# tencent-ailab/V-Express

Hardware: AMD Instinct MI355X
Metric: decoded frames/sec at 512x512, 25 DDIM steps (higher is better)
Workload: dtype bf16; 1 GPU; 512x512, 16 frames (1 window(s) of 16, overlap 4), 25 DDIM steps, CFG 3.5, random-init UNet3D + ReferenceNet banks + sd-vae-ft-mse decode; frames=16, windows=1, parallelism=window x CFG-half units over 1 GPU(s)

## Files before the change

v-express_amd/csrc/vx_attn.hip:

```cpp
#include "vx_common.h"
#include <stdio.h>
#include "../../include/vexpress_hip.h"

#include <stdlib.h>

#include <type_traits>

namespace {

struct AttnParams {
  const bf16_t* q; int ldq;
  const bf16_t* k; int ldk;
  const bf16_t* vt; int vt_pitch;
  bf16_t* out; int ldo;
  int batch, heads, n_q, n_kv, d, q_per_kv;
  float c;
  const float* kmax;
};

__device__ __forceinline__ int k_lds_off(int slab, int key, int grp) {
  return slab * 4096 + key * 64 + ((grp ^ ((0 - (key >> 2)) & 3)) << 4);
}
__device__ __forceinline__ int v_lds_off(int row, int chunk) { return row * 128 + ((chunk ^ ((row >> 1) & 7)) << 4); }

// ... 697 lines not shown
  };
  if (wide && (p.heads % 8) == 0 && KK * (p.f <= 16 ? 1 : 2) <= 6) {
    dim3 grid((unsigned)((waves + 7) / 8));
    name(p.f <= 16 ? 0 : 1, p.f <= 16 ? 1 : 2, 8);
    if (p.f <= 16) hipLaunchKernelGGL((temporal_attn_kernel<KK, DT, 1, 8>), grid, dim3(512), 0, stream, p);
    else hipLaunchKernelGGL((temporal_attn_kernel<KK, DT, 2, 8>), grid, dim3(512), 0, stream, p);
    return vx_check_launch("vx_temporal_attention");
  }
  dim3 grid((unsigned)((waves + 3) / 4));
  name(p.f <= 16 ? 2 : 3, p.f <= 16 ? 1 : 2, 4);
  if (p.f <= 16) hipLaunchKernelGGL((temporal_attn_kernel<KK, DT, 1, 4>), grid, dim3(256), 0, stream, p);
  else hipLaunchKernelGGL((temporal_attn_kernel<KK, DT, 2, 4>), grid, dim3(256), 0, stream, p);
  return vx_check_launch("vx_temporal_attention");
}

constexpr int SKV_MAX = 16;

__global__ __launch_bounds__(256) void small_kv_attn_kernel(const bf16_t* __restrict__ q, int ldq,
                                                            const bf16_t* __restrict__ kv, int ldkv, int v_off,
                                                            bf16_t* __restrict__ out, int ldo, int n_q, int n_kv,
                                                            int heads, int d, float c) {
  extern __shared__ __attribute__((aligned(16))) char smem[];
  bf16_t* kvs = reinterpret_cast<bf16_t*>(smem);
  const int C = heads * d;
  const int b = blockIdx.y;
  const int tid = threadIdx.x;
  const int cch = C >> 3;
  for (int idx = tid; idx < n_kv * 2 * cch; idx += 256) {
    int j = idx / (2 * cch), rem = idx % (2 * cch);
    int which = rem / cch, ch = (rem % cch) * 8;
    const bf16_t* src = kv + ((size_t)b * n_kv + j) * ldkv + (which ? v_off : 0) + ch;
    *reinterpret_cast<uint4*>(kvs + ((size_t)(j * 2 + which)) * C + ch) = *reinterpret_cast<const uint4*>(src);
  }
  __syncthreads();
  const long item = (long)blockIdx.x * 256 + tid;
  if (item >= (long)n_q * heads) return;
  const int h = (int)(item % heads);
  const int tok = (int)(item / heads);
  const bf16_t* qp = q + ((size_t)b * n_q + tok) * ldq + h * d;
  float sc[SKV_MAX];
#pragma unroll
  for (int j = 0; j < SKV_MAX; ++j) sc[j] = 0.f;
  for (int ch = 0; ch < d; ch += 8) {
    float qv[8];
    unpack_bf16x8(*reinterpret_cast<const uint4*>(qp + ch), qv);
#pragma unroll
    for (int j = 0; j < SKV_MAX; ++j) {
      if (j < n_kv) {
        float kvv[8];
        unpack_bf16x8(*reinterpret_cast<const uint4*>(kvs + (size_t)(j * 2) * C + h * d + ch), kvv);
#pragma unroll
        for (int e = 0; e < 8; ++e) sc[j] = fmaf(qv[e], kvv[e], sc[j]);
      }
    }
  }
  float mx = -INFINITY;
#pragma unroll
  for (int j = 0; j < SKV_MAX; ++j)
    if (j < n_kv) mx = fmaxf(mx, sc[j]);
  float den = 0.f;
#pragma unroll
  for (int j = 0; j < SKV_MAX; ++j) {
    float pv = (j < n_kv) ? __builtin_amdgcn_exp2f((sc[j] - mx) * c) : 0.f;
    sc[j] = pv;
    den += pv;
  }
  const float inv = 1.0f / den;
  bf16_t* op = out + ((size_t)b * n_q + tok) * ldo + h * d;
  for (int ch = 0; ch < d; ch += 8) {
    float acc[8] = {0.f, 0.f, 0.f, 0.f, 0.f, 0.f, 0.f, 0.f};
#pragma unroll
    for (int j = 0; j < SKV_MAX; ++j) {
      if (j < n_kv) {
        float vv[8];
        unpack_bf16x8(*reinterpret_cast<const uint4*>(kvs + (size_t)(j * 2 + 1) * C + h * d + ch), vv);
#pragma unroll
        for (int e = 0; e < 8; ++e) acc[e] = fmaf(sc[j], vv[e], acc[e]);
      }
    }
#pragma unroll
    for (int e = 0; e < 8; ++e) acc[e] *= inv;
    *reinterpret_cast<uint4*>(op + ch) = pack_bf16x8(acc);
  }
}

__global__ __launch_bounds__(256) void key_norm_max_kernel(const bf16_t* __restrict__ k, int ldk, int heads, int n_kv,
                                                           int d, float* __restrict__ out) {
  __shared__ float red[256];
  const int bh = blockIdx.x, b = bh / heads, h = bh - b * heads;
  const bf16_t* base = k + (size_t)b * n_kv * ldk + h * d;
  const int chunks = d >> 3;
  float best = 0.f;
  for (int key = threadIdx.x; key < n_kv; key += 256) {
    const bf16_t* row = base + (size_t)key * ldk;
    float ss = 0.f;
    for (int c = 0; c < chunks; ++c) {
      float f[8];
      unpack_bf16x8(*reinterpret_cast<const uint4*>(row + 8 * c), f);
#pragma unroll
      for (int e = 0; e < 8; ++e) ss = fmaf(f[e], f[e], ss);
    }
    best = fmaxf(best, ss);
  }
  red[threadIdx.x] = best;
  __syncthreads();
  for (int s = 128; s > 0; s >>= 1) {
    if ((int)threadIdx.x < s) red[threadIdx.x] = fmaxf(red[threadIdx.x], red[threadIdx.x + s]);
    __syncthreads();
  }
  if (threadIdx.x == 0) out[bh] = sqrtf(red[0]);
}

constexpr int KNM8_KEYS = 256;
__global__ __launch_bounds__(256) void key_norm_max8_kernel(const bf16_t* __restrict__ k, int ldk, int n_kv, int d,
                                                            float* __restrict__ out) {
  __shared__ float red[4][8];
  const int b = blockIdx.y, key0 = blockIdx.x * KNM8_KEYS;
  const int lane = threadIdx.x & 63, wave = threadIdx.x >> 6, h = lane & 7;
  const bf16_t* base = k + (size_t)b * n_kv * ldk + h * d;
  const int chunks = d >> 3;
  float best = 0.f;
  for (int kk = wave * 8 + (lane >> 3); kk < KNM8_KEYS; kk += 32) {
    const int key = min(key0 + kk, n_kv - 1);
    const bf16_t* row = base + (size_t)key * ldk;
    float ss = 0.f;
    for (int c = 0; c < chunks; ++c) {
      float f[8];
      unpack_bf16x8(*reinterpret_cast<const uint4*>(row + 8 * c), f);
#pragma unroll
      for (int e = 0; e < 8; ++e) ss = fmaf(f[e], f[e], ss);
    }
    best = fmaxf(best, ss);
  }
  best = fmaxf(best, __shfl_xor(best, 8, 64));
  best = fmaxf(best, __shfl_xor(best, 16, 64));
  best = fmaxf(best, __shfl_xor(best, 32, 64));
  if (lane < 8) red[wave][lane] = best;
  __syncthreads();
  if (threadIdx.x < 8) {
    const float m = fmaxf(fmaxf(red[0][threadIdx.x], red[1][threadIdx.x]), fmaxf(red[2][threadIdx.x], red[3][threadIdx.x]));
    atomicMax(reinterpret_cast<unsigned int*>(out) + b * 8 + threadIdx.x, __float_as_uint(sqrtf(m)));
  }
}

int attention_impl(const void* q, int ldq, const void* k, int ldk, const void* vt, int vt_pitch, void* out, int ldo,
                   int batch, int heads, int n_q, int n_kv, int head_dim, int q_per_kv, float scale,
                   const float* key_norm_max, hipStream_t stream);

}

int vx_attn3_variant();
int vx_attn3_launch(const void* q, int ldq, const void* k, int ldk, const void* vt, int vt_pitch, void* out, int ldo,
                    int batch, int heads, int n_q, int n_kv, int q_per_kv, float c, const float* kmax,
                    hipStream_t stream);

extern "C" int vx_key_norm_max(const void* k, int ldk, int kv_batches, int heads, int n_kv, int head_dim, float* out,
                               void* stream) {
  VX_REQUIRE(k && out, "vx_key_norm_max: null pointer");
  VX_REQUIRE(kv_batches > 0 && heads > 0 && n_kv > 0 && head_dim > 0 && (head_dim % 8) == 0 && (ldk % 8) == 0,
             "vx_key_norm_max: bad sizes (head_dim=%d ldk=%d)", head_dim, ldk);
  static int v8 = -1;
  if (v8 < 0) {
    const char* e = getenv("VX_KNM8");
    v8 = !(e && atoi(e) == 0);
  }
  if (v8 && heads == 8 && n_kv >= 2 * KNM8_KEYS && kv_batches <= 65535) {
    if (hipMemsetAsync(out, 0, (size_t)kv_batches * heads * sizeof(float), (hipStream_t)stream) != hipSuccess) {
      vx_set_error("vx_key_norm_max: hipMemsetAsync failed");
      return VX_ERR_HIP;
    }
    hipLaunchKernelGGL(key_norm_max8_kernel, dim3((n_kv + KNM8_KEYS - 1) / KNM8_KEYS, kv_batches), dim3(256), 0,
                       (hipStream_t)stream, (const bf16_t*)k, ldk, n_kv, head_dim, out);
    return vx_check_launch("vx_key_norm_max");
  }
  hipLaunchKernelGGL(key_norm_max_kernel, dim3(kv_batches * heads), dim3(256), 0, (hipStream_t)stream,
                     (const bf16_t*)k, ldk, heads, n_kv, head_dim, out);
  return vx_check_launch("vx_key_norm_max");
}

extern "C" int vx_attention(const void* q, int ldq, const void* k, int ldk, const void* vt, int vt_pitch, void* out,
                            int ldo, int batch, int heads, int n_q, int n_kv, int head_dim, int q_per_kv,
                            float scale, void* stream) {
  return attention_impl(q, ldq, k, ldk, vt, vt_pitch, out, ldo, batch, heads, n_q, n_kv, head_dim, q_per_kv, scale,
                        nullptr, (hipStream_t)stream);
}

extern "C" int vx_attention_bounded(const void* q, int ldq, const void* k, int ldk, const void* vt, int vt_pitch,
                                    void* out, int ldo, int batch, int heads, int n_q, int n_kv, int head_dim,
                                    int q_per_kv, float scale, const float* key_norm_max, void* stream) {
  VX_REQUIRE(key_norm_max != nullptr, "vx_attention_bounded: null key_norm_max");
  return attention_impl(q, ldq, k, ldk, vt, vt_pitch, out, ldo, batch, heads, n_q, n_kv, head_dim, q_per_kv, scale,
                        key_norm_max, (hipStream_t)stream);
}

namespace {
int attention_impl(const void* q, int ldq, const void* k, int ldk, const void* vt, int vt_pitch, void* out, int ldo,
                   int batch, int heads, int n_q, int n_kv, int head_dim, int q_per_kv, float scale,
                   const float* key_norm_max, hipStream_t stream) {
  VX_REQUIRE(q && k && vt && out, "vx_attention: null pointer");
  VX_REQUIRE(batch > 0 && heads > 0 && n_q > 0 && n_kv > 0 && q_per_kv > 0 && (batch % q_per_kv) == 0,
             "vx_attention: bad sizes");
  VX_REQUIRE((head_dim % 8) == 0 && (ldq % 8) == 0 && (ldk % 8) == 0 && (vt_pitch % 8) == 0 && (ldo % 4) == 0 &&
                 vt_pitch >= n_kv,
             "vx_attention: alignment (head_dim=%d ldq=%d ldk=%d pitch=%d ldo=%d)", head_dim, ldq, ldk, vt_pitch, ldo);
  VX_REQUIRE((long)batch * heads <= 65535, "vx_attention: batch*heads too large for grid.y");
  AttnParams p{(const bf16_t*)q, ldq, (const bf16_t*)k, ldk, (const bf16_t*)vt, vt_pitch, (bf16_t*)out, ldo,
               batch, heads, n_q, n_kv, head_dim, q_per_kv, scale == 0.f ? 1.0f : scale * 1.4426950408889634f,
               key_norm_max};
  VX_REQUIRE(scale >= 0.f, "vx_attention: scale must be positive (or 0: K carries scale * log2 e)");
  const int d = head_dim;
  static int v1 = -1;
  if (v1 < 0) v1 = getenv("VX_ATTN_V1") != nullptr;
  if (!v1 && d == 40 && key_norm_max && vx_attn3_variant() > 0 && ((size_t)n_kv * ldk * 2) < (1ull << 31) &&
      ((size_t)d * vt_pitch * 2) < (1ull << 31))
    return vx_attn3_launch(q, ldq, k, ldk, vt, vt_pitch, out, ldo, batch, heads, n_q, n_kv, q_per_kv, p.c, key_norm_max,
                           stream);
  if (!v1 && d > 32 && d <= 48 && (d % 16) != 0)
    return key_norm_max ? launch_attn2<2, 3, 2, true, true>(p, stream) : launch_attn2<2, 3, 2, true, false>(p, stream);
  if (d <= 32) return launch_attn<1, 2, 4, true>(p, stream);
  if (d <= 48) return launch_attn<2, 3, 2, true>(p, stream);
  if (d <= 64) return launch_attn<2, 4, 2, true>(p, stream);
  if (d <= 80) return launch_attn<3, 5, 2, true>(p, stream);
  if (d <= 96) return launch_attn<3, 6, 2, true>(p, stream);
  if (d <= 128) return launch_attn<4, 8, 2, true>(p, stream);
  if (d <= 160) return launch_attn<5, 10, 2, false>(p, stream);
  if (d == 512) return launch_attn<16, 32, 1, false, 1>(p, stream);
  vx_set_error("vx_attention: unsupported head_dim %d", d);
  return VX_ERR_UNSUPPORTED;
}
}

extern "C" int vx_temporal_attention(const void* qkv, int ldqkv, void* out, int ldo, int b, int f, int hw, int heads,
                                     int head_dim, float scale, void* stream_) {
  hipStream_t stream = (hipStream_t)stream_;
  VX_REQUIRE(qkv && out, "vx_temporal_attention: null pointer");
  VX_REQUIRE(f >= 1 && f <= 32, "vx_temporal_attention: f=%d outside [1,32] (PositionalEncoding max_len)", f);
  VX_REQUIRE((head_dim % 8) == 0 && (ldqkv % 8) == 0 && (ldo % 4) == 0, "vx_temporal_attention: alignment");
  TemporalParams p{(const bf16_t*)qkv, ldqkv, (bf16_t*)out, ldo, b, f, hw, heads, head_dim,
                   scale * 1.4426950408889634f};
  const int d = head_dim;
  if (d <= 32) return launch_temporal<1, 2>(p, stream);
  if (d <= 64) return launch_temporal<2, 4>(p, stream);
  if (d <= 96) return launch_temporal<3, 6>(p, stream);
  if (d <= 128) return launch_temporal<4, 8>(p, stream);
  if (d <= 160) return launch_temporal<5, 10>(p, stream);
  vx_set_error("vx_temporal_attention: unsupported head_dim %d", d);
  return VX_ERR_UNSUPPORTED;
}

extern "C" int vx_small_kv_attention(const void* q, int ldq, const void* kv, int ldkv, int v_off, void* out, int ldo,
                                     int batch, int n_q, int n_kv, int heads, int head_dim, float scale,
                                     void* stream_) {
  hipStream_t stream = (hipStream_t)stream_;
  VX_REQUIRE(q && kv && out, "vx_small_kv_attention: null pointer");
  VX_REQUIRE(n_kv >= 1 && n_kv <= SKV_MAX, "vx_small_kv_attention: n_kv=%d outside [1,%d]", n_kv, SKV_MAX);
  VX_REQUIRE((head_dim % 8) == 0 && (ldq % 8) == 0 && (ldkv % 8) == 0 && (v_off % 8) == 0 && (ldo % 8) == 0,
             "vx_small_kv_attention: alignment");
  const int C = heads * head_dim;
  size_t smem = (size_t)n_kv * 2 * C * sizeof(bf16_t);
  VX_REQUIRE(smem <= 64 * 1024, "vx_small_kv_attention: K/V tile %zu B exceeds LDS budget", smem);
  dim3 grid(ceil_div((long)n_q * heads, 256), batch);
  hipLaunchKernelGGL(small_kv_attn_kernel, grid, dim3(256), smem, stream, (const bf16_t*)q, ldq, (const bf16_t*)kv,
                     ldkv, v_off, (bf16_t*)out, ldo, n_q, n_kv, heads, head_dim, scale * 1.4426950408889634f);
  return vx_check_launch("vx_small_kv_attention");
}
```

v-express_amd/ops.py:

```python
import ctypes as C
import logging
import os

import torch

from . import lib as L

class _CurrentLib:

    def __getattr__(self, name):
        return getattr(L.current(), name)


_lib = _CurrentLib()


def __getattr__(name):
    if name == "BF16":
        return L.ELEM[0]
    raise AttributeError(name)


def _stream():
    return C.c_void_p(torch.cuda.current_stream().cuda_stream)
# ... 705 lines not shown
    p.wqkv_t, p.wo_t, p.colsum_p = (t.data_ptr() for t in hit[3:6])
    p.bias_o = bo.data_ptr() if bo is not None else None
    p.ln_stats = stats.data_ptr() if stats is not None else None
    p.stats_out = stats_out.data_ptr() if stats_out is not None else None
    p.ln_eps, p.scale = eps, (c // heads) ** -0.5
    with _hbm_op("tblock_fused", 2 * m * c * 2, flops=8.0 * m * c * c + 4.0 * m * f * c):
        L.check(_lib.vx_tblock_fused(C.byref(p), _stream()), "vx_tblock_fused")
    _set_gn(h)
    return h


def vt_pitch(n):
    return (n + 7) // 8 * 8


def gemm_split(a, w, bias, parts, *, part_cols, seq_len=0, head_dim=0, geom=None, ln=None):
    p, geom = _base_params(a, w, geom)
    p.epi = L.VX_EPI_SPLIT
    _set_ln(p, ln)
    p.bias = bias.data_ptr() if bias is not None else None
    p.part_cols, p.n_parts = part_cols, len(parts)
    p.seq_len, p.head_dim = seq_len, head_dim
    for i, (kind, t) in enumerate(parts):
        _chk_bf16(t, "part")
        p.part_out[i] = t.data_ptr()
        if kind == "rows":
            p.part_kind[i] = L.VX_PART_ROWS
            p.part_ld[i] = _row_stride(t)[0]
        else:
            p.part_kind[i] = L.VX_PART_VT
            p.part_ld[i] = 0
            p.vt_pitch = t.shape[-1]
            if not t.is_contiguous():
                raise ValueError("V^T destination must be contiguous")
    _launch_gemm(p, "vx_gemm(split)")


def alloc_vt(seqs, heads, head_dim, n, device):
    pitch = vt_pitch(n)
    if pitch != n:
        return torch.zeros((seqs, heads, head_dim, pitch), device=device, dtype=L.ELEM[0])
    return torch.empty((seqs, heads, head_dim, pitch), device=device, dtype=L.ELEM[0])


def _gn_slices(hw):
    return max(1, min(64, hw // 16))


_PADDED = {}


def padded_buffer(device, frames, H, W, c):
    key = (device, _stream_key(device), frames, H, W, c, L.ELEM[0])
    buf = _PADDED.get(key)
    if buf is None:
        buf = torch.zeros((frames, (H + 2) * (W + 2), c), device=device, dtype=L.ELEM[0])
        _PADDED[key] = buf
    return buf


def groupnorm(x1, gamma, beta, *, frames, hw, groups, eps, silu, x2=None, out=None, pad_hw=None):
    _chk_bf16(x1, "x1")
    if not x1.is_contiguous() or (x2 is not None and not x2.is_contiguous()):
        raise ValueError("groupnorm inputs must be contiguous")
    c1 = x1.shape[-1]
    c2 = x2.shape[-1] if x2 is not None else 0
    width, pad = hw, 0
    if pad_hw is not None:
        H, W = pad_hw
        if H * W != hw or out is not None:
            raise ValueError("pad_hw must factor hw and excludes `out`")
        out = padded_buffer(x1.device, frames, H, W, c1 + c2)
        width, pad = W, 1
    elif out is None:
        out = torch.empty((frames, hw, c1 + c2), device=x1.device, dtype=L.ELEM[0])
    slices = _gn_slices(hw)
    st = gn_of(x1) if x2 is None else None
    elems = frames * hw * (c1 + c2)
    if st is not None and st.fits(frames, hw, groups, c1):
        with _hbm_op("groupnorm_apply", 4 * elems):
            L.check(_lib.vx_groupnorm_apply(_ptr(x1), c1, None, 0, frames, hw, groups, float(eps), _ptr(gamma),
                                            _ptr(beta), int(silu), _ptr(out), _ptr(st.ws), st.slabs, slices, width, pad,
                                            _stream()), "vx_groupnorm_apply")
        return out
    ws = torch.empty(int(_lib.vx_groupnorm_ws_floats(frames, slices, groups)), device=x1.device,
                     dtype=torch.float32)
    with _hbm_op("groupnorm_stats+apply", 6 * elems):
        L.check(_lib.vx_groupnorm(_ptr(x1), c1, _ptr(x2), c2, frames, hw, groups, float(eps), _ptr(gamma), _ptr(beta),
                                  int(silu), _ptr(out), _ptr(ws), slices, width, pad, _stream()), "vx_groupnorm")
    return out


GN_FOLD = [os.environ.get("VX_GN_FOLD", "1") != "0" and os.environ.get("VX_GEMM_NOFAST") is None]


def gn_fold_applies(m, hw, c, n):
    items = _ITEMS[0]
    geom = (("c", c), ("n", n), ("hw", hw), ("rows_item", m // items if items and items > 0 and m % items == 0 else None))
    folded, applied = "GroupNorm folded into per-frame weights (no normalised tensor)", "GroupNorm apply pass + GEMM"
    if not GN_FOLD[0] or items is None or items <= 0 or m % items or hw % 256 or n % 320 or c % 64:
        return _note_path("groupnorm_proj_in", geom, False, applied, "fold off or geometry not whole 256 x 320 tiles per frame")
    if _ring_off(c):
        return _note_path("groupnorm_proj_in", geom, False, applied, "persistent kernel switched off")
    rows_item = m // items
    ok = rows_item % 256 == 0 and (2 * rows_item // 256) * (n // 320) >= 192 and n * 2 <= hw
    return _note_path("groupnorm_proj_in", geom, ok, folded if ok else applied,
                      "" if ok else "per-frame weight copies would cost more than the normalised tensor")


def groupnorm_stats(x1, *, frames, hw, groups, x2=None):
    _chk_bf16(x1, "x1")
    st = gn_of(x1) if x2 is None else None
    if st is not None and st.fits(frames, hw, groups, x1.shape[-1]):
        return st.ws, st.slabs
    if not x1.is_contiguous() or (x2 is not None and not x2.is_contiguous()):
        raise ValueError("groupnorm inputs must be contiguous")
    c1 = x1.shape[-1]
    c2 = x2.shape[-1] if x2 is not None else 0
    slices = _gn_slices(hw)
    ws = torch.empty(int(_lib.vx_groupnorm_ws_floats(frames, slices, groups)), device=x1.device, dtype=torch.float32)
    with _hbm_op("groupnorm_stats", 2 * frames * hw * (c1 + c2)):
        L.check(_lib.vx_groupnorm_stats(_ptr(x1), c1, _ptr(x2), c2, frames, hw, groups, _ptr(ws), slices, _stream()),
                "vx_groupnorm_stats")
    return ws, slices


def groupnorm_fold_linear(ws, gamma, w, bias_beta, *, frames, hw, groups, eps, slices=None):
    _chk_bf16(w, "w")
    n, c = w.shape
    if bias_beta.dtype != torch.float32 or gamma.dtype != torch.float32 or not w.is_contiguous():
        raise TypeError("groupnorm_fold_linear: float32 gamma / bias_beta, contiguous bf16 weight expected")
    w_f = torch.empty((frames, n, c), device=w.device, dtype=L.ELEM[0])
    b_f = torch.empty((frames, n), device=w.device, dtype=torch.float32)
    L.check(_lib.vx_groupnorm_fold_linear(_ptr(ws), frames, hw, slices or _gn_slices(hw), groups, float(eps), _ptr(gamma), c,
                                          _ptr(w), _ptr(bias_beta), n, _ptr(w_f), _ptr(b_f), _stream()),
            "vx_groupnorm_fold_linear")
    return w_f, b_f


def layernorm(x, gamma, beta, eps=1e-5, *, add=None, add_rows_per_entry=1, add_entries=1, out=None):
    _chk_bf16(x, "x")
    ldx, rows = _row_stride(x)
    c = x.shape[-1]
    if out is None:
        out = torch.empty((rows, c), device=x.device, dtype=L.ELEM[0])
    with _hbm_op("layernorm", 4 * rows * c):
        L.check(_lib.vx_layernorm(_ptr(x), ldx, rows, c, float(eps), _ptr(gamma), _ptr(beta), _ptr(add),
                                  add_rows_per_entry, add_entries, _ptr(out), _row_stride(out)[0], _stream()),
                "vx_layernorm")
    return out


_BOUNDED_SOFTMAX = [os.environ.get("VX_ATTN_BOUND", "1") != "0"]


def key_norm_max(k, *, kv_batches, heads, n_kv, head_dim):
    ldk, _ = _row_stride(k)
    out = torch.empty((kv_batches * heads,), device=k.device, dtype=torch.float32)
    with _hbm_op("key_norm_max", 2 * kv_batches * n_kv * heads * head_dim):
        L.check(_lib.vx_key_norm_max(_ptr(k), ldk, kv_batches, heads, n_kv, head_dim, _ptr(out), _stream()),
                "vx_key_norm_max")
    return out


def attention(q, k, vt, *, batch, heads, n_q, n_kv, head_dim, q_per_kv=1, out=None, kmax=None, k_prescaled=False):
    ldq, _ = _row_stride(q)
    ldk, _ = _row_stride(k)
    if out is None:
        out = torch.empty((batch * n_q, heads * head_dim), device=q.device, dtype=L.ELEM[0])
    scale = 0.0 if k_prescaled else head_dim ** -0.5
    c = heads * head_dim
    flops = 4.0 * batch * heads * n_q * n_kv * head_dim
    nbytes = 2 * (2 * batch * n_q * c + 2 * (batch // q_per_kv) * n_kv * c)
    if _BOUNDED_SOFTMAX[0] and 32 < head_dim <= 48 and head_dim % 16:
        if kmax is None:
            kmax = key_norm_max(k, kv_batches=batch // q_per_kv, heads=heads, n_kv=n_kv, head_dim=head_dim)
        with _hbm_op("attention", nbytes, flops=flops):
            L.check(_lib.vx_attention_bounded(_ptr(q), ldq, _ptr(k), ldk, _ptr(vt), vt.shape[-1], _ptr(out),
                                              _row_stride(out)[0], batch, heads, n_q, n_kv, head_dim, q_per_kv,
                                              scale, _ptr(kmax), _stream()), "vx_attention_bounded")
        return out
    with _hbm_op("attention", nbytes, flops=flops):
        L.check(_lib.vx_attention(_ptr(q), ldq, _ptr(k), ldk, _ptr(vt), vt.shape[-1], _ptr(out), _row_stride(out)[0],
                                  batch, heads, n_q, n_kv, head_dim, q_per_kv, scale, _stream()),
                "vx_attention")
    return out


def temporal_attention(qkv, *, b, f, hw, heads, head_dim, out=None):
    _chk_bf16(qkv, "qkv")
    ld, rows = _row_stride(qkv)
    if rows != b * f * hw:
        raise ValueError("qkv rows != b*f*hw")
    if out is None:
        out = torch.empty((rows, heads * head_dim), device=qkv.device, dtype=L.ELEM[0])
    with _hbm_op("temporal_attention", 2 * rows * 4 * heads * head_dim, flops=4.0 * rows * f * heads * head_dim):
        L.check(_lib.vx_temporal_attention(_ptr(qkv), ld, _ptr(out), _row_stride(out)[0], b, f, hw, heads, head_dim,
                                           head_dim ** -0.5, _stream()), "vx_temporal_attention")
    return out


def small_kv_attention(q, kv, *, batch, n_q, n_kv, heads, head_dim, out=None):
    ldq, _ = _row_stride(q)
    ldkv, _ = _row_stride(kv)
    c = heads * head_dim
    if out is None:
        out = torch.empty((batch * n_q, c), device=q.device, dtype=L.ELEM[0])
    with _hbm_op("small_kv_attention", 2 * (2 * batch * n_q * c + 2 * batch * n_kv * c)):
        L.check(_lib.vx_small_kv_attention(_ptr(q), ldq, _ptr(kv), ldkv, c, _ptr(out), _row_stride(out)[0], batch, n_q,
                                           n_kv, heads, head_dim, head_dim ** -0.5, _stream()),
                "vx_small_kv_attention")
    return out


UPSAMPLE_PHASES = [os.environ.get("VX_UPSAMPLE_PHASES", "1") != "0"]
UPSAMPLE_PHASES_MIN_HW = [int(os.environ.get("VX_UPSAMPLE_PHASES_MIN_HW", "256"))]


def upsample_phases_applies(H, W, c):
    geom = (("hw_in", H * W), ("c", c))
    four, one = "four 2x2 convolutions over the original image + interleave", "one 3x3 convolution with the upsampling in its gather"
    ok = UPSAMPLE_PHASES[0] and H * W >= UPSAMPLE_PHASES_MIN_HW[0] and c % 64 == 0
    return _note_path("upsample_conv", geom, ok, four if ok else one,
                      "" if ok else "switched off / input frame below VX_UPSAMPLE_PHASES_MIN_HW pixels / channels not a multiple of 64")


def pad_image(x, frames, H, W):
    _chk_bf16(x, "x")
    if not x.is_contiguous():
        raise ValueError("pad_image: contiguous input")
    c = x.shape[-1]
    out = padded_buffer(x.device, frames, H, W, c)
    L.check(_lib.vx_pad_image(_ptr(x), frames, H, W, c, _ptr(out), _stream()), "vx_pad_image")
    return out


def pixel_shuffle2x(phases, frames, H, W):
    _chk_bf16(phases, "phases")
    if phases.dim() != 3 or phases.shape[0] != 4 or phases.shape[1] != frames * H * W or not phases.is_contiguous():
        raise ValueError("pixel_shuffle2x: phases must be a contiguous [4, frames*H*W, C] tensor")
    c = phases.shape[-1]
    out = torch.empty((frames, 4 * H * W, c), device=phases.device, dtype=L.ELEM[0])
    L.check(_lib.vx_pixel_shuffle2x(_ptr(phases), phases.stride(0), frames, H, W, c, _ptr(out), _stream()), "vx_pixel_shuffle2x")
    return out


def upsample_conv_phases(x, w_phases, bias, *, frames, H, W):
    cout = w_phases.shape[1]
    xp = pad_image(x, frames, H, W)
    ph = torch.empty((4, frames * H * W, cout), device=x.device, dtype=L.ELEM[0])
    g = ConvGeom(frames, H + 2, W + 2, 2, 2, 1, 0, out_hw=(H, W))
    for a in (0, 1):
        for b in (0, 1):
            gemm(xp.view(frames * (H + 2) * (W + 2), -1), w_phases[a * 2 + b], bias, geom=g,
                 a_pixel_offset=a * (W + 2) + b, out=ph[a * 2 + b])
    return pixel_shuffle2x(ph, frames, H, W)


FF_PROJ_FOLD = [os.environ.get("VX_FF_PROJ_FOLD", "1") != "0"]
FF_PROJ_FOLD_MIN_HW = [int(os.environ.get("VX_FF_PROJ_FOLD_MIN_HW", "256"))]
FF_PROJ_FOLD_MM = [os.environ.get("VX_FF_PROJ_FOLD_MM", "1") != "0"]


def ff_proj_fold_applies(m, c, hidden):
    hw = _FRAME_ROWS[0]
    geom = (("c", c), ("hidden", hidden), ("hw", hw))
    one, two = "FF output GEMM + proj_out as one dual-source GEMM (K = 5C)", "two launches (FF output GEMM, proj_out)"
    if not FF_PROJ_FOLD[0] or FP8_PROJ[0]:
        return _note_path("ff_proj_out", geom, False, two, "switched off / fp8 projections")
    ok = hw is not None and hw >= FF_PROJ_FOLD_MIN_HW[0] and c % 64 == 0 and hidden % 64 == 0
    return _note_path("ff_proj_out", geom, ok, one if ok else two, "" if ok else "frame below VX_FF_PROJ_FOLD_MIN_HW rows")


AX_FUSED = [os.environ.get("VX_AX_FUSED", "1") != "0"]


class AudioFold:

    def __init__(self, kq, colsum, sbias, vo, frames, c):
        self.kq, self.colsum, self.sbias, self.vo, self.frames, self.c = kq, colsum, sbias, vo, frames, c


def audio_xattn_applies(c, heads, n_ctx, hw):
    geom = (("c", c), ("heads", heads), ("n_ctx", n_ctx), ("hw%16", hw % 16))
    one, three = "one launch (vx_audio_xattn)", "three launches (q GEMM + 5-key attention + output GEMM)"
    if not AX_FUSED[0] or not LN_FOLD[0] or FP8_PROJ[0]:
        return _note_path("audio_cross_attention", geom, False, three, "switched off / LayerNorm fold off / fp8 projections")
    ok = bool(_lib.vx_audio_xattn_supported(int(c), int(heads), int(n_ctx), int(hw)))
    return _note_path("audio_cross_attention", geom, ok, one if ok else three,
                      "" if ok else "the one-launch form is built for 8 heads, 5 audio tokens per frame, c % 320 == 0")


def audio_xattn_pack(kv, wq_folded, bq_folded, wo, *, frames, n_ctx, heads):
    _chk_bf16(kv, "kv")
    _chk_bf16(wq_folded, "wq")
    _chk_bf16(wo, "wo")
    c = wo.shape[0]
    if kv.shape != (frames * n_ctx, 2 * c) or tuple(wq_folded.shape) != (c, c) or tuple(wo.shape) != (c, c) or \
            not wq_folded.is_contiguous() or not wo.is_contiguous():
        raise ValueError("audio_xattn_pack: shapes")
    if bq_folded is not None and (bq_folded.dtype != torch.float32 or bq_folded.numel() != c):
        raise TypeError("audio_xattn_pack: folded bias must be float32 [C]")
    dev = kv.device
    kq = torch.empty((frames, 48 * c), device=dev, dtype=L.ELEM[0])
    vo = torch.empty((frames, 48 * c), device=dev, dtype=L.ELEM[0])
    cs = torch.empty((frames, 48), device=dev, dtype=torch.float32)
    sb = torch.empty((frames, 48), device=dev, dtype=torch.float32)
    L.check(_lib.vx_audio_xattn_pack(_ptr(kv), _row_stride(kv)[0], _ptr(wq_folded), _ptr(bq_folded), _ptr(wo), c, heads, n_ctx,
                                     frames, _ptr(kq), _ptr(cs), _ptr(sb), _ptr(vo), _stream()), "vx_audio_xattn_pack")
    return AudioFold(kq, cs, sb, vo, frames, c)


def audio_xattn(h, stats, fold, bias_o, alpha, *, rows_per_frame, stats_out=None, stats_eps=1e-5, out=None):
    _chk_bf16(h, "h")
    ldx, m = _row_stride(h)
    c = h.shape[-1]
    if out is None:
        out = h
    if m != fold.frames * rows_per_frame or c != fold.c:
        raise ValueError(f"audio_xattn: {m} rows of width {c} against operands for {fold.frames} frames x {rows_per_frame} rows, width {fold.c}")
    if stats.dtype != torch.float32 or not stats.is_contiguous() or tuple(stats.shape) not in ((m, 2), (m, 4)):
        raise ValueError("audio_xattn: stats must be a contiguous float32 [m, 2] / [m, 4] tensor")
    p = L.AxAttnParams()
    p.x, p.ldx, p.out, p.ldo = h.data_ptr(), ldx, out.data_ptr(), _row_stride(out)[0]
    p.rows, p.c, p.rows_per_frame = m, c, rows_per_frame
    p.ln_stats, p.ln_stats_parts, p.ln_eps = stats.data_ptr(), 2 if stats.shape[1] == 4 else 0, 1e-5
    p.kq, p.kq_colsum, p.kq_bias, p.vo = fold.kq.data_ptr(), fold.colsum.data_ptr(), fold.sbias.data_ptr(), fold.vo.data_ptr()
# ... 124 lines not shown
```

Baseline: 14.63 frames/s.

## Add bounded-softmax attention kernel for head dims 80 and 160

Adds a new attention kernel for head_dim 80 and 160 that uses a precomputed key-norm bound (Cauchy-Schwarz) as a fixed softmax shift instead of an online running max. It falls back to an exact two-pass max computation when the row sum underflows. This is meant to remove the per-tile rescaling work of online softmax in the deeper UNet levels when the key set is long. The cost is an extra key-norm-max kernel launch, and a possible fallback pass when the bound is too loose.

Result: no change. 14.74 frames/s, median of 6 (+0.8%).

```diff
diff --git a/v-express_amd/csrc/vx_attn.hip b/v-express_amd/csrc/vx_attn.hip
--- a/v-express_amd/csrc/vx_attn.hip
+++ b/v-express_amd/csrc/vx_attn.hip
@@ -873,6 +873,10 @@
 int vx_attn3_variant();
 int vx_attn3_launch(const void* q, int ldq, const void* k, int ldk, const void* vt, int vt_pitch, void* out, int ldo,
                     int batch, int heads, int n_q, int n_kv, int q_per_kv, float c, const float* kmax,
+                    hipStream_t stream);
+bool vx_attnw_supports(int head_dim);
+int vx_attnw_launch(const void* q, int ldq, const void* k, int ldk, const void* vt, int vt_pitch, void* out, int ldo,
+                    int batch, int heads, int n_q, int n_kv, int head_dim, int q_per_kv, float c, const float* kmax,
                     hipStream_t stream);
 
 extern "C" int vx_key_norm_max(const void* k, int ldk, int kv_batches, int heads, int n_kv, int head_dim, float* out,
@@ -936,6 +940,10 @@
       ((size_t)d * vt_pitch * 2) < (1ull << 31))
     return vx_attn3_launch(q, ldq, k, ldk, vt, vt_pitch, out, ldo, batch, heads, n_q, n_kv, q_per_kv, p.c, key_norm_max,
                            stream);
+  if (!v1 && key_norm_max && vx_attnw_supports(d) && ((size_t)n_kv * ldk * 2) < (1ull << 31) &&
+      ((size_t)d * vt_pitch * 2) < (1ull << 31))
+    return vx_attnw_launch(q, ldq, k, ldk, vt, vt_pitch, out, ldo, batch, heads, n_q, n_kv, d, q_per_kv, p.c, key_norm_max,
+                           stream);
   if (!v1 && d > 32 && d <= 48 && (d % 16) != 0)
     return key_norm_max ? launch_attn2<2, 3, 2, true, true>(p, stream) : launch_attn2<2, 3, 2, true, false>(p, stream);
   if (d <= 32) return launch_attn<1, 2, 4, true>(p, stream);
diff --git a/v-express_amd/csrc/vx_attnw.hip b/v-express_amd/csrc/vx_attnw.hip
--- /dev/null
+++ b/v-express_amd/csrc/vx_attnw.hip
@@ -0,0 +1,328 @@
+#include "vx_common.h"
+#include "vx_gemm_common.h"
+
+#include <type_traits>
+
+namespace {
+
+struct AttnWParams {
+  const bf16_t* q; int ldq;
+  const bf16_t* k; int ldk;
+  const bf16_t* vt; int vt_pitch;
+  bf16_t* out; int ldo;
+  int batch, heads, n_q, n_kv, q_per_kv;
+  float c;
+  const float* kmax;
+};
+
+constexpr int AW_QT = 2;
+
+__device__ __forceinline__ int aw_pi16(int r) { return 32 * (r >> 5) + 8 * ((r >> 2) & 3) + 4 * ((r >> 4) & 1) + (r & 3); }
+
+template <int D>
+struct AttnWShape {
+  static_assert(D % 16 == 0 && D >= 64, "attnw: head dim must be a multiple of 16");
+  static constexpr int NKF = D / 32;
+  static constexpr bool HALF = (D % 32) != 0;
+  static constexpr int KK = NKF + (HALF ? 1 : 0);
+  static constexpr int DT = D / 16;
+  static constexpr int HK = NKF * 4096;
+  static constexpr int V = HK + (HALF ? 2048 : 0);
+  static constexpr int STAGE = V + D * 128;
+  static constexpr int NPIECE = STAGE / 1024;
+  static constexpr int PPW = NPIECE / 4;
+  static constexpr int NKP = NKF * 4 + (HALF ? 2 : 0);
+  static_assert(NPIECE % 4 == 0, "attnw: pieces must split evenly over the 4 waves");
+};
+
+template <int D>
+__device__ __forceinline__ uint32_t aw_piece_src(int pw, int lane, int t, bool edge, int ldk, int vt_pitch, int n_kv) {
+  using S = AttnWShape<D>;
+  if (pw < S::NKP) {
+    int r, col;
+    if (pw < 4 * S::NKF) {
+      const int kk = pw >> 2;
+      r = 16 * (pw & 3) + (lane >> 2);
+      col = 32 * kk + 8 * ((lane & 3) ^ ((0 - (r >> 2)) & 3));
+    } else {
+      r = 32 * (pw - 4 * S::NKF) + (lane >> 1);
+      col = 32 * S::NKF + 8 * (lane & 1);
+    }
+    int key = t * 64 + aw_pi16(r);
+    if (edge) key = min(key, n_kv - 1);
+    return ((uint32_t)key * (uint32_t)ldk + (uint32_t)col) * 2u;
+  }
+  const int r = 8 * (pw - S::NKP) + (lane >> 3), chunk = (lane & 7) ^ ((r >> 1) & 7);
+  const int c = (edge && t * 64 + 8 * chunk >= n_kv) ? 0 : chunk;
+  return ((uint32_t)r * (uint32_t)vt_pitch + (uint32_t)(t * 64 + 8 * c)) * 2u;
+}
+
+template <int D, bool UNIT, int MINW>
+__global__ __launch_bounds__(256, MINW) void attnw_kernel(const AttnWParams p) {
+  using S = AttnWShape<D>;
+  constexpr int NBUF = 2, KK = S::KK, DT = S::DT, PPW = S::PPW;
+  constexpr bool SHIFT_IN_MFMA = S::HALF;
+  extern __shared__ __attribute__((aligned(16))) char smem[];
+  const int tid = threadIdx.x, lane = tid & 63;
+  const int wave = __builtin_amdgcn_readfirstlane(tid >> 6);
+  const int i = lane & 15, g = lane >> 4;
+  const int nqb = (p.n_q + 64 * AW_QT - 1) / (64 * AW_QT);
+  const int lid = xcd_remap(blockIdx.x, gridDim.x);
+  const int bh = lid / nqb, qb = lid - bh * nqb;
+  const int b = bh / p.heads, h = bh - b * p.heads;
+  const int kvb = b / p.q_per_kv;
+  const int q0 = qb * (64 * AW_QT) + wave * (16 * AW_QT);
+  const bf16_t* __restrict__ kbase = p.k + (size_t)kvb * p.n_kv * p.ldk + h * D;
+  const bf16_t* __restrict__ vbase = p.vt + (size_t)(kvb * p.heads + h) * D * p.vt_pitch;
+  const int n_tiles = (p.n_kv + 63) >> 6;
+  const bool ragged = (p.n_kv & 63) != 0;
+
+  uint32_t src0[PPW];
+#pragma unroll
+  for (int s = 0; s < PPW; ++s) src0[s] = aw_piece_src<D>(wave + 4 * s, lane, 0, false, p.ldk, p.vt_pitch, p.n_kv);
+  const uint32_t kstep = 128u * (uint32_t)p.ldk, vstep = 128u;
+  const uint32_t lds0 = lds_addr_of(smem);
+  auto issue = [&](int t) {
+    const uint32_t so = lds0 + (uint32_t)(t % NBUF) * S::STAGE;
+    const bool edge = ragged && t == n_tiles - 1;
+#pragma unroll
+    for (int s = 0; s < PPW; ++s) {
+      const int pw = wave + 4 * s;
+      const bool is_k = pw < S::NKP;
+      const uint32_t off = edge ? aw_piece_src<D>(pw, lane, t, true, p.ldk, p.vt_pitch, p.n_kv)
+                                : src0[s] + (uint32_t)t * (is_k ? kstep : vstep);
+      glds16_s(is_k ? (const void*)kbase : (const void*)vbase, off, so + (uint32_t)pw * 1024u);
+    }
+  };
+
+  uint4 qf[AW_QT][KK];
+  float mfix[AW_QT];
+#pragma unroll
+  for (int qt = 0; qt < AW_QT; ++qt) {
+    const int qrow = q0 + 16 * qt + i;
+    float ss = 0.f;
+#pragma unroll
+    for (int kk = 0; kk < KK; ++kk) {
+      const int dcol = 32 * kk + 8 * g;
+      uint4 v = make_uint4(0, 0, 0, 0);
+      if (qrow < p.n_q && dcol < D) {
+        v = *reinterpret_cast<const uint4*>(p.q + (size_t)(b * p.n_q + qrow) * p.ldq + h * D + dcol);
+        float f[8];
+        unpack_bf16x8(v, f);
+#pragma unroll
+        for (int e = 0; e < 8; ++e) ss = fmaf(f[e], f[e], ss);
+      }
+      qf[qt][kk] = v;
+    }
+    ss = wave_xor_sum(ss, 16);
+    ss = wave_xor_sum(ss, 32);
+    mfix[qt] = sqrtf(ss) * p.kmax[kvb * p.heads + h] - (UNIT ? VX_P_HEADROOM : VX_P_HEADROOM / p.c);
+  }
+  float mc[AW_QT];
+  auto set_shift = [&](const float (&m)[AW_QT]) {
+#pragma unroll
+    for (int qt = 0; qt < AW_QT; ++qt) {
+      if constexpr (SHIFT_IN_MFMA) {
+        if (g == 2) qf[qt][KK - 1] = make_uint4((uint32_t)f32_to_bf16(-m[qt]), 0, 0, 0);
+      } else {
+        mc[qt] = UNIT ? -m[qt] : -m[qt] * p.c;
+      }
+    }
+  };
+
+  const int a_k0 = i * 64 + ((g ^ ((0 - (i >> 2)) & 3)) << 4);
+  const int a_kh = S::HK + i * 32 + ((g & 1) << 4);
+  const int vx = (i >> 1) & 7;
+  const int a_v0 = S::V + i * 128 + ((g ^ vx) << 4);
+  const int a_v1 = S::V + i * 128 + (((4 | g) ^ vx) << 4);
+
+  f32x4_t o[DT][AW_QT];
+  float lsum[AW_QT];
+  auto zero_o = [&]() {
+#pragma unroll
+    for (int qt = 0; qt < AW_QT; ++qt) {
+      lsum[qt] = 0.f;
+#pragma unroll
+      for (int dt = 0; dt < DT; ++dt) o[dt][qt] = f32x4_t{0.f, 0.f, 0.f, 0.f};
+    }
+  };
+
+  auto qk = [&](f32x4_t (&s_)[4][AW_QT], int t) {
+    const char* st = smem + (t % NBUF) * S::STAGE;
+#pragma unroll
+    for (int kt = 0; kt < 4; ++kt) {
+#pragma unroll
+      for (int qt = 0; qt < AW_QT; ++qt) s_[kt][qt] = f32x4_t{0.f, 0.f, 0.f, 0.f};
+#pragma unroll
+      for (int kk = 0; kk < KK; ++kk) {
+        uint4 kf;
+        if (S::HALF && kk == KK - 1) {
+          kf = *reinterpret_cast<const uint4*>(st + a_kh + kt * 512);
+          if (g == 2) kf.x = VX_E16_ONE;
+        } else {
+          kf = *reinterpret_cast<const uint4*>(st + a_k0 + kk * 4096 + kt * 1024);
+        }
+#pragma unroll
+        for (int qt = 0; qt < AW_QT; ++qt) s_[kt][qt] = mfma16(kf, qf[qt][kk], s_[kt][qt]);
+      }
+    }
+  };
+  auto mask = [&](f32x4_t (&s_)[4][AW_QT], int t) {
+#pragma unroll
+    for (int kt = 0; kt < 4; ++kt)
+#pragma unroll
+      for (int r = 0; r < 4; ++r)
+        if (t * 64 + 32 * (kt >> 1) + 8 * g + 4 * (kt & 1) + r >= p.n_kv) {
+#pragma unroll
+          for (int qt = 0; qt < AW_QT; ++qt) s_[kt][qt][r] = -INFINITY;
+        }
+  };
+  auto expo = [&](f32x4_t (&s_)[4][AW_QT]) {
+#pragma unroll
+    for (int qt = 0; qt < AW_QT; ++qt) {
+      float part[4];
+#pragma unroll
+      for (int kt = 0; kt < 4; ++kt) {
+#pragma unroll
+        for (int r = 0; r < 4; ++r) {
+          float x = s_[kt][qt][r];
+          if constexpr (SHIFT_IN_MFMA) x = UNIT ? x : x * p.c;
+          else x = UNIT ? x + mc[qt] : fmaf(x, p.c, mc[qt]);
+          s_[kt][qt][r] = __builtin_amdgcn_exp2f(x);
+        }
+        part[kt] = (s_[kt][qt][0] + s_[kt][qt][1]) + (s_[kt][qt][2] + s_[kt][qt][3]);
+      }
+      lsum[qt] += (part[0] + part[1]) + (part[2] + part[3]);
+    }
+  };
+  auto pv = [&](const f32x4_t (&s_)[4][AW_QT], int t) {
+    const char* st = smem + (t % NBUF) * S::STAGE;
+#pragma unroll
+    for (int ks_ = 0; ks_ < 2; ++ks_) {
+      uint4 pb[AW_QT];
+#pragma unroll
+      for (int qt = 0; qt < AW_QT; ++qt) {
+        const f32x4_t& a = s_[2 * ks_][qt];
+        const f32x4_t& c2 = s_[2 * ks_ + 1][qt];
+        pb[qt] = make_uint4(pack_bf16x2(a[0], a[1]), pack_bf16x2(a[2], a[3]), pack_bf16x2(c2[0], c2[1]),
+                            pack_bf16x2(c2[2], c2[3]));
+      }
+      const char* vp = st + (ks_ ? a_v1 : a_v0);
+#pragma unroll
+      for (int dt = 0; dt < DT; ++dt) {
+        const uint4 vf = *reinterpret_cast<const uint4*>(vp + dt * 2048);
+#pragma unroll
+        for (int qt = 0; qt < AW_QT; ++qt) o[dt][qt] = mfma16(vf, pb[qt], o[dt][qt]);
+      }
+    }
+  };
+
+  float mrun[AW_QT];
+  auto run = [&](auto maxpass_c) {
+    constexpr bool MAXPASS = decltype(maxpass_c)::value;
+    __syncthreads();
+    issue(0);
+    for (int t = 0; t < n_tiles; ++t) {
+      asm volatile("s_waitcnt vmcnt(0)" ::: "memory");
+      __syncthreads();
+      if (t + 1 < n_tiles) issue(t + 1);
+      f32x4_t cur[4][AW_QT];
+      qk(cur, t);
+      if (ragged && t == n_tiles - 1) mask(cur, t);
+      if (MAXPASS) {
+#pragma unroll
+        for (int qt = 0; qt < AW_QT; ++qt) {
+          float mx = mrun[qt];
+#pragma unroll
+          for (int kt = 0; kt < 4; ++kt)
+            mx = fmaxf(fmaxf(fmaxf(mx, cur[kt][qt][0]), fmaxf(cur[kt][qt][1], cur[kt][qt][2])), cur[kt][qt][3]);
+          mrun[qt] = mx;
+        }
+      } else {
+        expo(cur);
+        pv(cur, t);
+      }
+    }
+  };
+  auto row_sum = [&](int qt) -> float { return wave_xor_sum(wave_xor_sum(lsum[qt], 16), 32); };
+
+  set_shift(mfix);
+  float l[AW_QT];
+  for (bool exact = false;; exact = true) {
+    zero_o();
+    run(std::false_type{});
+    bool bad = false;
+#pragma unroll
+    for (int qt = 0; qt < AW_QT; ++qt) {
+      l[qt] = row_sum(qt);
+      bad |= (q0 + 16 * qt + i < p.n_q) && !(l[qt] >= VX_P_MIN_ROWSUM(p.n_kv));
+    }
+    if (exact) break;
+    __syncthreads();
+    const bool wave_bad = __builtin_amdgcn_ballot_w64(bad) != 0;
+    if (lane == 0) reinterpret_cast<int*>(smem)[wave] = wave_bad;
+    __syncthreads();
+    const int* flags = reinterpret_cast<const int*>(smem);
+    if (!(flags[0] | flags[1] | flags[2] | flags[3])) break;
+    const float zero[AW_QT] = {0.f, 0.f};
+    set_shift(zero);
+#pragma unroll
+    for (int qt = 0; qt < AW_QT; ++qt) mrun[qt] = -INFINITY;
+    run(std::true_type{});
+#pragma unroll
+    for (int qt = 0; qt < AW_QT; ++qt) mrun[qt] = wave_rows_max(mrun[qt]);
+    set_shift(mrun);
+  }
+
+#pragma unroll
+  for (int qt = 0; qt < AW_QT; ++qt) {
+    const float inv = 1.0f / l[qt];
+    const int qrow = q0 + 16 * qt + i;
+    if (qrow >= p.n_q) continue;
+    bf16_t* orow = p.out + (size_t)(b * p.n_q + qrow) * p.ldo + h * D;
+#pragma unroll
+    for (int dt = 0; dt < DT; ++dt) {
+      uint2 w;
+      w.x = pack_bf16x2(o[dt][qt][0] * inv, o[dt][qt][1] * inv);
+      w.y = pack_bf16x2(o[dt][qt][2] * inv, o[dt][qt][3] * inv);
+      *reinterpret_cast<uint2*>(orow + 16 * dt + 4 * g) = w;
+    }
+  }
+}
+
+template <int D, bool UNIT, int MINW>
+int launch_attnw(const AttnWParams& p, hipStream_t stream) {
+  constexpr int smem = 2 * AttnWShape<D>::STAGE;
+  auto kern = attnw_kernel<D, UNIT, MINW>;
+  static bool attr_set = false;
+  if (!attr_set) {
+    hipError_t e = hipFuncSetAttribute((const void*)kern, hipFuncAttributeMaxDynamicSharedMemorySize, smem);
+    if (e != hipSuccess) {
+      vx_set_error("vx_attention: hipFuncSetAttribute(%d) failed: %s", smem, hipGetErrorString(e));
+      return VX_ERR_HIP;
+    }
+    attr_set = true;
+  }
+  dim3 grid((unsigned)((long)ceil_div(p.n_q, 64 * AW_QT) * p.batch * p.heads));
+  static char sym[64] = "";
+  if (!sym[0]) snprintf(sym, sizeof(sym), "attnw_kernel<%d, %s, %d>", D, UNIT ? "true" : "false", MINW);
+  g_vx_last_kernel = sym;
+  hipLaunchKernelGGL(kern, grid, dim3(256), smem, stream, p);
+  return vx_check_launch("vx_attention");
+}
+
+}
+
+bool vx_attnw_supports(int head_dim) { return head_dim == 80 || head_dim == 160; }
+
+int vx_attnw_launch(const void* q, int ldq, const void* k, int ldk, const void* vt, int vt_pitch, void* out, int ldo,
+                    int batch, int heads, int n_q, int n_kv, int head_dim, int q_per_kv, float c, const float* kmax,
+                    hipStream_t stream) {
+  AttnWParams p{(const bf16_t*)q, ldq, (const bf16_t*)k, ldk, (const bf16_t*)vt, vt_pitch, (bf16_t*)out, ldo,
+                batch, heads, n_q, n_kv, q_per_kv, c, kmax};
+  const bool unit = c == 1.0f;
+  if (head_dim == 80) return unit ? launch_attnw<80, true, 3>(p, stream) : launch_attnw<80, false, 3>(p, stream);
+  if (head_dim == 160) return unit ? launch_attnw<160, true, 2>(p, stream) : launch_attnw<160, false, 2>(p, stream);
+  vx_set_error("vx_attention: attnw has no head_dim %d", head_dim);
+  return VX_ERR_UNSUPPORTED;
+}
diff --git a/v-express_amd/ops.py b/v-express_amd/ops.py
--- a/v-express_amd/ops.py
+++ b/v-express_amd/ops.py
@@ -881,6 +881,22 @@
 
 
 _BOUNDED_SOFTMAX = [os.environ.get("VX_ATTN_BOUND", "1") != "0"]
+_BOUNDED_SOFTMAX_WIDE = [os.environ.get("VX_ATTN_BOUND_WIDE", "1") != "0"]
+BOUNDED_WIDE_MIN_KV = 256
+
+
+def _bounded_path(head_dim, n_kv):
+    if not _BOUNDED_SOFTMAX[0]:
+        return False
+    if 32 < head_dim <= 48 and head_dim % 16:
+        return True
+    if head_dim in (80, 160):
+        wide = _BOUNDED_SOFTMAX_WIDE[0] and n_kv >= BOUNDED_WIDE_MIN_KV
+        _note_path("attention", (("head_dim", head_dim), ("n_kv", n_kv)), wide,
+                   "bounded softmax (attnw)" if wide else "online softmax (attn_kernel)",
+                   "" if wide else ("switched off" if not _BOUNDED_SOFTMAX_WIDE[0] else "short key set"))
+        return wide
+    return False
 
 
 def key_norm_max(k, *, kv_batches, heads, n_kv, head_dim):
@@ -901,7 +917,7 @@
     c = heads * head_dim
     flops = 4.0 * batch * heads * n_q * n_kv * head_dim
     nbytes = 2 * (2 * batch * n_q * c + 2 * (batch // q_per_kv) * n_kv * c)
-    if _BOUNDED_SOFTMAX[0] and 32 < head_dim <= 48 and head_dim % 16:
+    if _bounded_path(head_dim, n_kv):
         if kmax is None:
             kmax = key_norm_max(k, kv_batches=batch // q_per_kv, heads=heads, n_kv=n_kv, head_dim=head_dim)
         with _hbm_op("attention", nbytes, flops=flops):
```
